# fhausmann/deepgrp

Measured on AMD Instinct MI355X. Metric: Mbp/sec predicted (whole node) at window=200 stride=50, 5-class, higher is better.
Workload: dtype f16

## Files before the change

deepgrp_amd/csrc/api.hip:

```cpp
#include "dgrp_model.h"

#include <stdarg.h>
#include <string.h>

#include <algorithm>
#include <vector>
#include <mutex>

static thread_local char g_err[512] = "";

void dgrp_set_error(const char *fmt, ...)
{
    va_list ap;
    va_start(ap, fmt);
    vsnprintf(g_err, sizeof(g_err), fmt, ap);
    va_end(ap);
}

DGRP_EXPORT int dgrp_abi_version(void) { return DGRP_ABI_VERSION; }
DGRP_EXPORT const char *dgrp_last_error(void) { return g_err; }

DGRP_EXPORT int dgrp_device_info(char *name, size_t name_cap, int *cu_count, int64_t *hbm_bytes)
{
    int dev = 0;
// ... 175 lines not shown
    m->onercp = 0;
    m->UP = (m->u + 31) / 32 * 32; m->NW = m->UP / 32; m->KS = m->UP / 16; m->nfrag = 0;
    m->d_pack = nullptr; m->d_ffb = nullptr; m->d_scale = nullptr; m->d_wtop = nullptr; m->d_raw = nullptr;
    m->d_pack_lo = nullptr; m->precision = 1; m->d_pack16 = nullptr; m->d_xtab = nullptr; m->d_stream = nullptr;
    m->d_packw = nullptr; m->d_xtabw = nullptr; m->NU16 = 0;
    const hipError_t e = upload_raw(m, kernel, rec, bias, nbias, ffk, nffk, ffb, scale);
    if (e != hipSuccess) {
        dgrp_set_error("dgrp_model_create: %s", hipGetErrorString(e));
        dgrp_model_destroy(m);
        return DGRP_EHIP;
    }
    *out = m;
    return DGRP_OK;
}

DGRP_EXPORT int dgrp_model_create(dgrp_model **out, int T, int u, int C, int attention, const float *kernel,
                                  const float *rec, const float *bias, const float *scale, const float *ffk,
                                  const float *ffb)
{
    DGRP_REQUIRE(out, "dgrp_model_create: NULL out");
    *out = nullptr;
    DGRP_REQUIRE(T >= 1 && T <= 65535, "dgrp_model_create: window size %d out of range", T);
    DGRP_REQUIRE(u >= 1 && u <= 2048, "dgrp_model_create: units=%d not supported (1..2048)", u);
    DGRP_REQUIRE(C >= 2 && C <= DGRP_MAXC, "dgrp_model_create: classes=%d not supported (2..%d)", C, DGRP_MAXC);
    DGRP_REQUIRE(kernel && rec && bias && ffk && ffb && (!attention || scale), "dgrp_model_create: NULL tensor");
    char nm[8];
    int rc = dgrp_device_info(nm, sizeof(nm), nullptr, nullptr);
    if (rc != DGRP_OK) return rc;

    dgrp_model *m = new dgrp_model();
    m->T = T; m->u = u; m->C = C; m->attention = attention ? 1 : 0;
    m->cell = 0;
    m->ref_only = 0; m->is_view = 0;
    if (u > 256 || C > 16) return create_ref_only(out, m, kernel, rec, bias, 2 * 3 * (int64_t)u, ffk, (int64_t)(attention ? 2 : 1) * u * C, ffb,
                                        attention ? scale : nullptr);
    m->UP = (u + 31) / 32 * 32;
    m->NW = m->UP / 32;
    m->KS = m->UP / 16;
    m->nfrag = 3 * (m->KS + 1) + 3;
    m->d_pack = nullptr; m->d_ffb = nullptr; m->d_scale = nullptr; m->d_wtop = nullptr; m->d_raw = nullptr;
    m->d_pack_lo = nullptr; m->precision = 0; m->d_pack16 = nullptr; m->d_xtab = nullptr; m->d_stream = nullptr;
    m->d_packw = nullptr; m->d_xtabw = nullptr; m->NU16 = 0;
    const int KS = m->KS, NF = m->nfrag, u3 = 3 * u;
    {
        double worst = 0.0;
        for (int j = 0; j < u; ++j) {
            double bz = 1.0, bg = 0.0;
            double kz = 0.0, kg = 0.0;
            for (int c = 0; c < 5; ++c) {
                kz = std::max(kz, (double)fabsf(kernel[(size_t)c * u3 + j]));
                kg = std::max(kg, (double)fabsf(kernel[(size_t)c * u3 + 2 * u + j]));
            }
            double sz = kz + fabs((double)bias[j] + (double)bias[u3 + j]);
            double sg = kg + fabsf(bias[2 * u + j]) + fabsf(bias[u3 + 2 * u + j]);
            for (int k = 0; k < u; ++k) {
                sz += fabsf(rec[(size_t)k * u3 + j]);
                sg += fabsf(rec[(size_t)k * u3 + 2 * u + j]);
            }
            bz += 1.4426950408889634 * sz;
            bg += 2.8853900817779268 * sg;
            if (!(bz + bg <= worst)) worst = bz + bg;
        }
        const char *safe = getenv("DGRP_GRU_SAFE");
        m->onercp = (m->NW <= 4 && worst <= 120.0 && !(safe && safe[0] == '1')) ? 1 : 0;
    }

    std::vector<uint16_t> pack((size_t)m->NW * NF * 64 * 8, 0);
    frag_writer fw{ pack, NF };
    for (int w = 0; w < m->NW; ++w) {
        for (int l = 0; l < 64; ++l) {
            const int unit = 32 * w + (l & 31);
            const bool uok = unit < u;
            for (int g = 0; g < 3; ++g) {
                const float gs = g < 2 ? -1.4426950408889634f : 2.8853900817779268f;
                pack_recurrent(fw, w, l, g * (KS + 1), KS, rec, u3, g * u + unit, u, uok, gs);
                float v8[8] = { 0, 0, 0, 0, 0, 0, 0, 0 };
                if (uok) {
                    for (int j = 0; j < 5; ++j) v8[j] = g < 2 ? gs * kernel[(size_t)j * u3 + g * u + unit] : 0.0f;
                    v8[5] = gs * (g < 2 ? (float)((double)bias[g * u + unit] + (double)bias[u3 + g * u + unit]) : bias[u3 + 2 * u + unit]);
                    if (m->onercp && g == 0) v8[5] += 1.0f;
                }
                pack_input(fw, w, l, g * (KS + 1) + KS, v8);
            }
            float x8[8] = { 0, 0, 0, 0, 0, 0, 0, 0 };
            if (uok) {
                for (int j = 0; j < 5; ++j) x8[j] = 2.8853900817779268f * kernel[(size_t)j * u3 + 2 * u + unit];
                x8[5] = 2.8853900817779268f * bias[2 * u + unit];
            }
            pack_input(fw, w, l, 3 * (KS + 1), x8);
            pack_dense(fw, w, l, 3 * (KS + 1) + 1, 3 * (KS + 1) + 2, ffk, attention ? u : 0, u, C);
        }
    }
    float ffb16[16] = { 0 };
    for (int c = 0; c < C; ++c) ffb16[c] = ffb[c];

#define CREATE_HIP(call)                                                                   \
    do {                                                                                   \
        hipError_t e_ = (call);                                                            \
        if (e_ != hipSuccess) {                                                            \
            dgrp_set_error("%s failed: %s", #call, hipGetErrorString(e_));                 \
            dgrp_model_destroy(m);                                                         \
            return DGRP_EHIP;                                                              \
        }                                                                                  \
    } while (0)
    CREATE_HIP(hipMalloc((void **)&m->d_pack, pack.size() * 2));
    CREATE_HIP(hipMemcpy(m->d_pack, pack.data(), pack.size() * 2, hipMemcpyHostToDevice));
    CREATE_HIP(hipMalloc((void **)&m->d_ffb, sizeof(ffb16)));
    CREATE_HIP(hipMemcpy(m->d_ffb, ffb16, sizeof(ffb16), hipMemcpyHostToDevice));
    if (attention) {
        std::vector<float> sc(m->UP, 0.0f), wtop((size_t)m->UP * 16, 0.0f);
        for (int k = 0; k < u; ++k) {
            sc[k] = scale[k];
            for (int c = 0; c < C; ++c) wtop[(size_t)k * 16 + c] = ffk[(size_t)k * C + c];
        }
        CREATE_HIP(hipMalloc((void **)&m->d_scale, sc.size() * 4));
        CREATE_HIP(hipMemcpy(m->d_scale, sc.data(), sc.size() * 4, hipMemcpyHostToDevice));
        CREATE_HIP(hipMalloc((void **)&m->d_wtop, wtop.size() * 4));
        CREATE_HIP(hipMemcpy(m->d_wtop, wtop.data(), wtop.size() * 4, hipMemcpyHostToDevice));
    }
    CREATE_HIP(upload_raw(m, kernel, rec, bias, 2 * (int64_t)u3, ffk, (int64_t)(attention ? 2 : 1) * u * C, ffb,
                          attention ? scale : nullptr));
    if (m->NW <= 4) {
        std::vector<uint16_t> lo((size_t)m->NW * 3 * KS * 64 * 8, 0);
        static const int order[3] = { 1, 2, 0 };
        for (int w = 0; w < m->NW; ++w)
            for (int ks = 0; ks < KS; ++ks)
                for (int gi = 0; gi < 3; ++gi) {
                    const int g = order[gi];
                    const float gs = g < 2 ? -1.4426950408889634f : 2.8853900817779268f;
                    for (int l = 0; l < 64; ++l) {
                        const int unit = 32 * w + (l & 31);
                        for (int j = 0; j < 8; ++j) {
                            const int k = 16 * ks + 8 * (l >> 5) + j;
                            uint16_t v = 0;
                            if (unit < u && k < u) {
                                const float x = gs * rec[(size_t)k * u3 + g * u + unit];
                                v = f2h(x - h2f(f2h(x)));
                            }
                            lo[((((size_t)w * KS + ks) * 3 + gi) * 64 + l) * 8 + j] = v;
                        }
                    }
            }
        CREATE_HIP(hipMalloc((void **)&m->d_pack_lo, lo.size() * 2));
        CREATE_HIP(hipMemcpy(m->d_pack_lo, lo.data(), lo.size() * 2, hipMemcpyHostToDevice));
        if (m->NW == 4) {
            static const int order16[3] = { 1, 2, 0 };
            std::vector<uint16_t> p16((size_t)4 * 48 * 64 * 8, 0);
            for (int w = 0; w < 4; ++w)
                for (int gi = 0; gi < 3; ++gi)
                    for (int ks = 0; ks < 4; ++ks)
                        for (int uh = 0; uh < 2; ++uh)
                            for (int l = 0; l < 64; ++l)
                                for (int j = 0; j < 8; ++j) {
                                    const int g = order16[gi], unit = 32 * w + 16 * uh + (l & 15), k = 32 * ks + 8 * (l >> 4) + j;
                                    uint16_t hi = 0, lo16 = 0;
                                    if (unit < u && k < u) {
                                        const float gs = g < 2 ? -1.4426950408889634f : 2.8853900817779268f;
                                        const float x = gs * rec[(size_t)k * u3 + g * u + unit];
                                        hi = f2h(x);
                                        lo16 = f2h(x - h2f(hi));
                                    }
                                    const size_t f = (size_t)gi * 8 + ks * 2 + uh;
                                    p16[(((size_t)w * 48 + f) * 64 + l) * 8 + j] = hi;
                                    p16[(((size_t)w * 48 + 24 + f) * 64 + l) * 8 + j] = lo16;
                                }
            std::vector<float> xt((size_t)5 * 4 * 128, 0.0f);
            const double cs = -1.4426950408889634, ch = 2.8853900817779268;
            for (int b = 0; b < 5; ++b)
                for (int unit = 0; unit < u; ++unit) {
                    float *row = &xt[(size_t)b * 512];
                    row[0 * 128 + unit] = (float)(cs * ((double)kernel[(size_t)b * u3 + u + unit] + (double)bias[u + unit] + (double)bias[u3 + u + unit]));
                    row[1 * 128 + unit] = (float)(ch * (double)bias[u3 + 2 * u + unit]);
                    row[2 * 128 + unit] = (float)(cs * ((double)kernel[(size_t)b * u3 + unit] + (double)bias[unit] + (double)bias[u3 + unit]) + (m->onercp ? 1.0 : 0.0));
                    row[3 * 128 + unit] = (float)(ch * ((double)kernel[(size_t)b * u3 + 2 * u + unit] + (double)bias[2 * u + unit]));
                }
            CREATE_HIP(hipMalloc((void **)&m->d_pack16, p16.size() * 2));
            CREATE_HIP(hipMemcpy(m->d_pack16, p16.data(), p16.size() * 2, hipMemcpyHostToDevice));
            CREATE_HIP(hipMalloc((void **)&m->d_xtab, xt.size() * 4));
            CREATE_HIP(hipMemcpy(m->d_xtab, xt.data(), xt.size() * 4, hipMemcpyHostToDevice));
        }
        if (u <= 64) {
            const int NU = (u + 15) / 16, KSw = (NU + 1) / 2, UP16 = 16 * NU, NFw = 6 * KSw * NU;
            auto wave_col = [](int c) { const int j = c / 32, q = (c % 32) / 8, sub = c % 8; return 16 * (2 * j + (sub >= 4 ? 1 : 0)) + 4 * q + (sub & 3); };
            static const int orderw[3] = { 1, 2, 0 };
            std::vector<uint16_t> pw((size_t)(NFw + 2 * KSw) * 64 * 8, 0);
            for (int gi = 0; gi < 3; ++gi)
                for (int ks = 0; ks < KSw; ++ks)
                    for (int ug = 0; ug < NU; ++ug)
                        for (int l = 0; l < 64; ++l)
                            for (int j = 0; j < 8; ++j) {
                                const int g = orderw[gi], unit = 16 * ug + (l & 15), k = wave_col(32 * ks + 8 * (l >> 4) + j);
                                if (unit >= u || k >= u) continue;
                                const float gs = g < 2 ? -1.4426950408889634f : 2.8853900817779268f;
                                const float x = gs * rec[(size_t)k * u3 + g * u + unit];
                                const uint16_t hi = f2h(x);
                                pw[((size_t)((gi * KSw + ks) * NU + ug) * 64 + l) * 8 + j] = hi;
                                pw[((size_t)(((3 + gi) * KSw + ks) * NU + ug) * 64 + l) * 8 + j] = f2h(x - h2f(hi));
                            }
            const int drow0 = attention ? u : 0;
            for (int ks = 0; ks < KSw; ++ks)
                for (int l = 0; l < 64; ++l)
                    for (int j = 0; j < 8; ++j) {
                        const int k = wave_col(32 * ks + 8 * (l >> 4) + j), c = l & 15;
                        if (k >= u || c >= C) continue;
                        const float v = 0.5f * ffk[(size_t)(drow0 + k) * C + c];
                        const uint16_t hi = f2h(v);
                        pw[((size_t)(NFw + 2 * ks) * 64 + l) * 8 + j] = hi;
                        pw[((size_t)(NFw + 2 * ks + 1) * 64 + l) * 8 + j] = f2h(v - h2f(hi));
                    }
            std::vector<float> xt((size_t)5 * 4 * UP16, 0.0f);
            const double cs = -1.4426950408889634, ch = 2.8853900817779268;
            for (int b = 0; b < 5; ++b)
                for (int unit = 0; unit < u; ++unit) {
                    float *row = &xt[(size_t)b * 4 * UP16];
                    row[0 * UP16 + unit] = (float)(cs * ((double)kernel[(size_t)b * u3 + u + unit] + (double)bias[u + unit] + (double)bias[u3 + u + unit]));
                    row[1 * UP16 + unit] = (float)(ch * (double)bias[u3 + 2 * u + unit]);
                    row[2 * UP16 + unit] = (float)(cs * ((double)kernel[(size_t)b * u3 + unit] + (double)bias[unit] + (double)bias[u3 + unit]) + (m->onercp ? 1.0 : 0.0));
                    row[3 * UP16 + unit] = (float)(ch * ((double)kernel[(size_t)b * u3 + 2 * u + unit] + (double)bias[2 * u + unit]));
                }
            CREATE_HIP(hipMalloc((void **)&m->d_packw, pw.size() * 2));
            CREATE_HIP(hipMemcpy(m->d_packw, pw.data(), pw.size() * 2, hipMemcpyHostToDevice));
            CREATE_HIP(hipMalloc((void **)&m->d_xtabw, xt.size() * 4));
            CREATE_HIP(hipMemcpy(m->d_xtabw, xt.data(), xt.size() * 4, hipMemcpyHostToDevice));
            m->NU16 = NU;
        }
        const char *pe = getenv("DGRP_GRU_PRECISION");
        m->precision = !(pe && pe[0] == '0') ? 1 : 0;
    }
    if (m->NW > 4) {
        static const float gs3[3] = { -1.4426950408889634f, -1.4426950408889634f, 2.8853900817779268f };
        CREATE_HIP(upload_stream(m, rec, 3, gs3));
        {
            const int UPm = m->UP;
            std::vector<float> xt((size_t)5 * 4 * UPm, 0.0f);
            const double cs = -1.4426950408889634, ch = 2.8853900817779268;
            for (int b = 0; b < 5; ++b)
                for (int unit = 0; unit < u; ++unit) {
                    float *row = &xt[(size_t)b * 4 * UPm];
                    row[0 * UPm + unit] = (float)(cs * ((double)kernel[(size_t)b * u3 + u + unit] + (double)bias[u + unit] + (double)bias[u3 + u + unit]));
                    row[1 * UPm + unit] = (float)(ch * (double)bias[u3 + 2 * u + unit]);
                    row[2 * UPm + unit] = (float)(cs * ((double)kernel[(size_t)b * u3 + unit] + (double)bias[unit] + (double)bias[u3 + unit]));
                    row[3 * UPm + unit] = (float)(ch * ((double)kernel[(size_t)b * u3 + 2 * u + unit] + (double)bias[2 * u + unit]));
                }
            CREATE_HIP(hipMalloc((void **)&m->d_xtab, xt.size() * 4));
            CREATE_HIP(hipMemcpy(m->d_xtab, xt.data(), xt.size() * 4, hipMemcpyHostToDevice));
        }
        const char *pe = getenv("DGRP_GRU_PRECISION");
        m->precision = !(pe && pe[0] == '0') ? 1 : 0;
    }
#undef CREATE_HIP
    *out = m;
    return DGRP_OK;
}

DGRP_EXPORT int dgrp_model_create_lstm(dgrp_model **out, int T, int u, int C, const float *kernel, const float *rec,
                                       const float *bias, const float *ffk, const float *ffb)
{
    DGRP_REQUIRE(out, "dgrp_model_create_lstm: NULL out");
    *out = nullptr;
    DGRP_REQUIRE(T >= 1 && T <= 65535, "dgrp_model_create_lstm: window size %d out of range", T);
    DGRP_REQUIRE(u >= 1 && u <= 2048, "dgrp_model_create_lstm: units=%d not supported (1..2048)", u);
    DGRP_REQUIRE(C >= 2 && C <= DGRP_MAXC, "dgrp_model_create_lstm: classes=%d not supported (2..%d)", C, DGRP_MAXC);
    DGRP_REQUIRE(kernel && rec && bias && ffk && ffb, "dgrp_model_create_lstm: NULL tensor");
    char nm[8];
    int rc = dgrp_device_info(nm, sizeof(nm), nullptr, nullptr);
    if (rc != DGRP_OK) return rc;
    dgrp_model *m = new dgrp_model();
    m->T = T; m->u = u; m->C = C; m->attention = 0; m->cell = 1;
    m->ref_only = 0; m->is_view = 0;
    if (u > 256 || C > 16) return create_ref_only(out, m, kernel, rec, bias, 4 * (int64_t)u, ffk, (int64_t)u * C, ffb, nullptr);
    m->UP = (u + 31) / 32 * 32;
    m->NW = m->UP / 32;
    m->KS = m->UP / 16;
    m->nfrag = 4 * (m->KS + 1) + 2;
    m->d_pack = nullptr; m->d_ffb = nullptr; m->d_scale = nullptr; m->d_wtop = nullptr; m->d_raw = nullptr;
    m->d_pack_lo = nullptr; m->precision = 0; m->d_pack16 = nullptr; m->d_xtab = nullptr; m->d_stream = nullptr;
    m->d_packw = nullptr; m->d_xtabw = nullptr; m->NU16 = 0;
    const int KS = m->KS, NF = m->nfrag, u4 = 4 * u;
    std::vector<uint16_t> pack((size_t)m->NW * NF * 64 * 8, 0);
    frag_writer fw{ pack, NF };
    for (int w = 0; w < m->NW; ++w)
        for (int l = 0; l < 64; ++l) {
            const int unit = 32 * w + (l & 31);
            const bool uok = unit < u;
            for (int g = 0; g < 4; ++g) {
                const float gs = g == 2 ? 2.8853900817779268f : -1.4426950408889634f;
                pack_recurrent(fw, w, l, g * (KS + 1), KS, rec, u4, g * u + unit, u, uok, gs);
                float v8[8] = { 0, 0, 0, 0, 0, 0, 0, 0 };
                if (uok) {
                    for (int j = 0; j < 5; ++j) v8[j] = gs * kernel[(size_t)j * u4 + g * u + unit];
                    v8[5] = gs * bias[g * u + unit];
                }
                pack_input(fw, w, l, g * (KS + 1) + KS, v8);
            }
            pack_dense(fw, w, l, 4 * (KS + 1), 4 * (KS + 1) + 1, ffk, 0, u, C);
        }
    float ffb16[16] = { 0 };
    for (int c = 0; c < C; ++c) ffb16[c] = ffb[c];
    hipError_t e = hipMalloc((void **)&m->d_pack, pack.size() * 2);
    if (e == hipSuccess) e = hipMemcpy(m->d_pack, pack.data(), pack.size() * 2, hipMemcpyHostToDevice);
    if (e == hipSuccess) e = hipMalloc((void **)&m->d_ffb, sizeof(ffb16));
    if (e == hipSuccess) e = hipMemcpy(m->d_ffb, ffb16, sizeof(ffb16), hipMemcpyHostToDevice);
    if (e == hipSuccess) e = upload_raw(m, kernel, rec, bias, u4, ffk, (int64_t)u * C, ffb, nullptr);
    if (e == hipSuccess) {
        static const float gs4[4] = { -1.4426950408889634f, -1.4426950408889634f, 2.8853900817779268f, -1.4426950408889634f };
        e = upload_stream(m, rec, 4, gs4);
        const char *pe = getenv("DGRP_GRU_PRECISION");
// ... 528 lines not shown
```

deepgrp_amd/csrc/gru_split2.hip:

```cpp
#include "gru_shared.h"
#include <mutex>
#include <type_traits>

typedef unsigned u32x4 __attribute__((ext_vector_type(4)));

namespace {

constexpr int NW = 4, UP = 128, KS = 4, HPAD = 16, HS = UP + HPAD;
constexpr int XT_PITCH = 4 * 128 * 4 + 32;

struct split2_weights {
    u32x4 hi[3][KS][2], lo[3][KS][2];
    u32x4 Bd_hi, Bd_lo;
};

#define LOAD2(a, pa, b, pb)                                                                                             \
    asm volatile("global_load_dwordx4 %0, %2, off\n\tglobal_load_dwordx4 %1, %3, off\n\ts_waitcnt vmcnt(0)"            \
                 : "=&a"(a), "=&a"(b) : "v"(pa), "v"(pb) : "memory")

#define MFMA_R(acc, Wf, b) asm volatile("v_mfma_f32_16x16x32_f16 %0, %1, %2, %0" : "+v"(acc) : "a"(Wf), "v"(b))
#define MFMA_D(acc, a, Wf) asm volatile("v_mfma_f32_16x16x32_f16 %0, %1, %2, %0" : "+v"(acc) : "v"(a), "a"(Wf))
#define MFMA_DZ(acc, a, Wf) asm volatile("v_mfma_f32_16x16x32_f16 %0, %1, %2, 0" : "=&v"(acc) : "v"(a), "a"(Wf))

struct tile_state {
    gru_params p;
    wg_ctx ctx;
    unsigned hcur, hnxt, lcur, lnxt;
    unsigned myseq;
    float h[16];
    f32x4 ar[4], ag[4], az[4], ax[4];
    f32x4 dpl;
    unsigned tabf, tabr;
    half8 f0h[2], f0l[2];
    int p_off;
    int64_t p_row0;
    bool pr_on;
};

template <int MODE, bool ONERCP>
__global__ void __launch_bounds__(256) __attribute__((amdgpu_waves_per_eu(1, 1))) gru_split2_kernel(const gru_params pin, int half_bytes)
{
    extern __shared__ __attribute__((aligned(16))) unsigned char smem[];
    const int tid = threadIdx.x;
    const int lane = tid & 63;
    const int wave = __builtin_amdgcn_readfirstlane(tid >> 6);
    const int T = pin.T, C = pin.C;

    split2_weights W;
    {
        const uint4 *p16 = pin.pack16 + (size_t)wave * 48 * 64 + lane;
#pragma unroll
        for (int g = 0; g < 3; ++g)
#pragma unroll
            for (int ks = 0; ks < KS; ++ks) {
                LOAD2(W.hi[g][ks][0], p16 + (size_t)(g * 8 + ks * 2) * 64, W.hi[g][ks][1], p16 + (size_t)(g * 8 + ks * 2 + 1) * 64);
                LOAD2(W.lo[g][ks][0], p16 + (size_t)(24 + g * 8 + ks * 2) * 64, W.lo[g][ks][1], p16 + (size_t)(24 + g * 8 + ks * 2 + 1) * 64);
            }
        const uint4 *mypack = pin.pack + (size_t)wave * pin.nfrag * 64 + lane;
        LOAD2(W.Bd_hi, mypack + (size_t)(3 * (2 * KS + 1) + 1) * 64, W.Bd_lo, mypack + (size_t)(3 * (2 * KS + 1) + 2) * 64);
    }
    for (int i = tid; i < 5 * 512; i += 256)
        *reinterpret_cast<float *>(smem + pin.xtab_off + (i / 512) * XT_PITCH + (i % 512) * 4) = pin.xtab[i];

    const int wi = lane & 15, q4 = lane >> 4;
    const int cls = lane & 15;
    const float fbias = cls < C ? pin.ffb[cls] : 0.0f;
    const int pwi = 4 * (lane >> 4) + wave;
    const unsigned frag_lane = (unsigned)(wi * HS + 8 * q4) * 2;
    const unsigned dense_lane = (unsigned)(wi * HS + 32 * wave + 8 * q4) * 2;
    const unsigned pub_lane = (unsigned)(wi * HS + 32 * wave + 4 * q4) * 2;
    const unsigned tab_lane = (unsigned)pin.xtab_off + (unsigned)(32 * wave + 4 * q4) * 4;

    tile_state S0, S1;
    auto setup = [&](tile_state &Z, int x) {
        unsigned char *base = smem + (size_t)x * half_bytes;
        _Float16 *lbuf = reinterpret_cast<_Float16 *>(base + pin.lo_tile_off);
        for (int i = tid; i < 32 * HS; i += 256) lbuf[i] = (_Float16)0.0f;
        Z.p = pin;
        const int64_t bid = wg_record_at<MODE>(pin, Z.p, 2 * (int64_t)blockIdx.x + x);
        Z.ctx = wg_setup<NW, MODE, HPAD>(Z.p, base, bid);
        Z.hcur = (unsigned)x * half_bytes;
        Z.hnxt = Z.hcur + 32 * HS * 2;
        Z.lcur = (unsigned)x * half_bytes + pin.lo_tile_off;
        Z.lnxt = Z.lcur + 32 * HS * 2;
        Z.myseq = (unsigned)(Z.ctx.seqs - smem) + wi * pin.Tp;
#pragma unroll
        for (int i = 0; i < 16; ++i) Z.h[i] = ONERCP ? -1.0f : 0.0f;
        Z.p_off = Z.ctx.rowoff[pwi];
        Z.p_row0 = Z.ctx.row0s[pwi];
        Z.pr_on = cls < C && pwi < Z.ctx.nvalid;
    };
    setup(S0, 0);
    setup(S1, 1);

    auto lds16 = [&](unsigned off) -> half8 { return *reinterpret_cast<const half8 *>(smem + off); };
    auto ldsf4 = [&](unsigned off) -> f32x4 { return *reinterpret_cast<const f32x4 *>(smem + off); };
    auto tab_rows = [&](tile_state &Z, uint32_t bf, uint32_t br) {
        bf = bf < 4 ? bf : 4;
        br = br < 4 ? 3 - br : 4;
        Z.tabf = tab_lane + bf * XT_PITCH;
        Z.tabr = tab_lane + br * XT_PITCH;
    };
    auto acc_init = [&](tile_state &Z, int g, int sub) {
        const f32x4 v = ldsf4(((sub & 1) ? Z.tabr : Z.tabf) + g * 512 + (sub >> 1) * 64);
        if (g == 0) Z.ar[sub] = v; else if (g == 1) Z.ag[sub] = v; else Z.az[sub] = v;
    };

    struct frag_ring { half8 h[2][2], l[2][2]; };
    struct dense_ops { half8 a0, a1, l0, l1; };
    struct fin_state { float d[NW], lg, m, e, s; };
    auto phase = [&](auto do_x, auto do_y, auto do_f, tile_state &X, tile_state &Y, int tx, int ty) __attribute__((always_inline)) {
        constexpr bool DO_X = decltype(do_x)::value, DO_Y = decltype(do_y)::value, DO_F = decltype(do_f)::value;
        frag_ring F;
        dense_ops D;
        fin_state fs;
        split_gate_tmp gt[16];
        float pbh[4][4];
        uint2 pbhv[4], pblv[4];
        uint32_t xp_bf = 4, xp_br = 4;
        const int td = ty - 1;
        const int tf = tx - 2;
        if constexpr (DO_X) { F.h[0][0] = X.f0h[0]; F.h[0][1] = X.f0h[1]; F.l[0][0] = X.f0l[0]; F.l[0][1] = X.f0l[1]; }
#define GAP __builtin_amdgcn_sched_barrier(0);
#define M_K(ks, n)                                                                                               \
    if constexpr (DO_X) {                                                                                        \
        constexpr int ps_ = (n) / 12, g_ = ((n) % 12) / 4, uh_ = ((n) % 4) / 2, rh_ = (n) % 2, sub_ = 2 * uh_ + rh_; \
        const half8 &b_ = ps_ == 1 ? F.l[(ks) & 1][rh_] : F.h[(ks) & 1][rh_];                                    \
        const u32x4 &w_ = ps_ == 2 ? W.lo[g_][ks][uh_] : W.hi[g_][ks][uh_];                                      \
        if constexpr (g_ == 0) MFMA_R(X.ar[sub_], w_, b_);                                                       \
        else if constexpr (g_ == 1) MFMA_R(X.ag[sub_], w_, b_);                                                  \
        else MFMA_R(X.az[sub_], w_, b_);                                                                         \
    }
#define M_D(i)                                                                                                   \
    if constexpr (DO_X) {                                                                                        \
        if constexpr ((i) == 0) MFMA_DZ(X.dpl, D.a0, W.Bd_hi);                                                   \
        else if constexpr ((i) == 1) MFMA_D(X.dpl, D.a1, W.Bd_hi);                                               \
        else if constexpr ((i) == 2) MFMA_D(X.dpl, D.a0, W.Bd_lo);                                               \
        else if constexpr ((i) == 3) MFMA_D(X.dpl, D.a1, W.Bd_lo);                                               \
        else if constexpr ((i) == 4) MFMA_D(X.dpl, D.l0, W.Bd_hi);                                               \
        else MFMA_D(X.dpl, D.l1, W.Bd_hi);                                                                       \
    }
#define PF(ks)                                                                                                   \
    if constexpr (DO_X) {                                                                                        \
        F.h[(ks) & 1][0] = lds16(X.hcur + frag_lane + 64 * (ks)); F.h[(ks) & 1][1] = lds16(X.hcur + frag_lane + 16 * HS * 2 + 64 * (ks)); \
        F.l[(ks) & 1][0] = lds16(X.lcur + frag_lane + 64 * (ks)); F.l[(ks) & 1][1] = lds16(X.lcur + frag_lane + 16 * HS * 2 + 64 * (ks)); \
    }
#define RDD                                                                                                      \
    if constexpr (DO_X) {                                                                                        \
        D.a0 = lds16(X.hcur + dense_lane); D.a1 = lds16(X.hcur + dense_lane + 16 * HS * 2);                      \
        D.l0 = lds16(X.lcur + dense_lane); D.l1 = lds16(X.lcur + dense_lane + 16 * HS * 2);                      \
        if (MODE == 2 && tx > 0 && (lane & 15) < X.ctx.nvalid)                                                   \
            split_avg_store(X.p, X.ctx.wg_w, tx - 1, UP, wave, D.a0, D.a1, D.l0, D.l1);                          \
    }
#define AXL(sub) \
    if constexpr (DO_Y) Y.ax[sub] = ldsf4((((sub) & 1) ? Y.tabr : Y.tabf) + 3 * 512 + ((sub) >> 1) * 64);
#define DS(i)                                                                                                    \
    if constexpr (DO_Y) Y.ctx.dpart[((size_t)(td & 1) * 4 * NW + wave) * 64 + lane + (i) * NW * 64] = Y.dpl[i];
#define G(e, op) \
    if constexpr (DO_Y) split_gate_op<ONERCP, op>(gt[e], Y.ar[(e) / 4][(e) % 4], Y.ag[(e) / 4][(e) % 4], Y.az[(e) / 4][(e) % 4], Y.ax[(e) / 4][(e) % 4], Y.h[e]);
#define PB(g, op)                                                                                                \
    if constexpr (DO_Y) {                                                                                        \
        if constexpr ((op) == 0) {                                                                               \
            pbh[g][0] = split_state_h<ONERCP>(Y.h[4 * (g)]); pbh[g][1] = split_state_h<ONERCP>(Y.h[4 * (g) + 1]); \
            pbh[g][2] = split_state_h<ONERCP>(Y.h[4 * (g) + 2]); pbh[g][3] = split_state_h<ONERCP>(Y.h[4 * (g) + 3]); \
        } else if constexpr ((op) == 1) {                                                                        \
            pbhv[g] = split_pack4(pbh[g]);                                                                       \
        } else if constexpr ((op) == 2) {                                                                        \
            split_residual4(pbh[g], pbhv[g]);                                                                    \
        } else if constexpr ((op) == 3) {                                                                        \
            pblv[g] = split_pack4(pbh[g]);                                                                       \
        } else {                                                                                                 \
            *reinterpret_cast<uint2 *>(smem + Y.hnxt + pub_lane + ((g) & 1) * 16 * HS * 2 + ((g) >> 1) * 32) = pbhv[g]; \
            *reinterpret_cast<uint2 *>(smem + Y.lnxt + pub_lane + ((g) & 1) * 16 * HS * 2 + ((g) >> 1) * 32) = pblv[g]; \
        }                                                                                                        \
    }
#define BAR                                                                                                      \
    if constexpr (DO_Y) {                                                                                        \
        asm volatile("s_waitcnt lgkmcnt(0)\n\ts_barrier" ::: "memory");                                          \
        unsigned sw_ = Y.hcur; Y.hcur = Y.hnxt; Y.hnxt = sw_;                                                    \
        sw_ = Y.lcur; Y.lcur = Y.lnxt; Y.lnxt = sw_;                                                             \
    }
#define RD0                                                                                                      \
    if constexpr (DO_Y) {                                                                                        \
        Y.f0h[0] = lds16(Y.hcur + frag_lane); Y.f0h[1] = lds16(Y.hcur + frag_lane + 16 * HS * 2);                \
        Y.f0l[0] = lds16(Y.lcur + frag_lane); Y.f0l[1] = lds16(Y.lcur + frag_lane + 16 * HS * 2);                \
    }
#define XP(op)                                                                                                   \
    if constexpr (DO_Y) {                                                                                        \
        if constexpr ((op) == 0) { xp_bf = smem[Y.myseq + ty + 1]; xp_br = smem[Y.myseq + T - 2 - ty]; }                       \
        else tab_rows(Y, xp_bf, xp_br);                                                                          \
    }
#define CI(g, sub) \
    if constexpr (DO_Y) acc_init(Y, g, sub);
#define FN(op)                                                                                                   \
    if constexpr (DO_F) {                                                                                        \
        if constexpr ((op) == 0) {                                                                               \
            const float *dp_ = X.ctx.dpart + ((size_t)(tf & 1) * 4 + wave) * NW * 64 + lane;                     \
            fs.d[0] = dp_[0]; fs.d[1] = dp_[64]; fs.d[2] = dp_[128]; fs.d[3] = dp_[192];                         \
        } else if constexpr ((op) == 1) {                                                                        \
            const float sum_ = ((fs.d[0] + fs.d[1]) + fs.d[2]) + fs.d[3];                                        \
            fs.lg = cls < C ? sum_ + fbias : -INFINITY;                                                          \
        } else if constexpr ((op) == 2) { if (MODE != 2) fs.m = row_max_ror<8>(fs.lg); }                         \
        else if constexpr ((op) == 3) { if (MODE != 2) fs.m = row_max_ror<4>(fs.m); }                            \
        else if constexpr ((op) == 4) { if (MODE != 2) fs.m = row_max_ror<2>(fs.m); }                            \
        else if constexpr ((op) == 5) { if (MODE != 2) fs.m = row_max_ror<1>(fs.m); }                            \
        else if constexpr ((op) == 6) { if (MODE != 2) fs.e = __builtin_amdgcn_exp2f(1.4426950408889634f * (fs.lg - fs.m)); } \
        else if constexpr ((op) == 7) { if (MODE != 2) fs.s = fs.e + row_ror<8>(fs.e); }                         \
        else if constexpr ((op) == 8) { if (MODE != 2) fs.s += row_ror<4>(fs.s); }                               \
        else if constexpr ((op) == 9) { if (MODE != 2) fs.s += row_ror<2>(fs.s); }                               \
        else if constexpr ((op) == 10) { if (MODE != 2) fs.s += row_ror<1>(fs.s); }                              \
        else if constexpr ((op) == 11) { if (MODE != 2) fs.e *= __builtin_amdgcn_rcpf(fs.s); }                   \
        else { if (X.pr_on && tf >= 0) emit_value<MODE>(X.p, X.ctx, X.p_off, X.p_row0, tf, cls, MODE == 2 ? fs.lg : fs.e); } \
    }
#include "gru_split2_phase.inc"
#undef GAP
#undef M_K
#undef M_D
#undef PF
#undef RDD
#undef AXL
#undef DS
#undef G
#undef PB
#undef BAR
#undef RD0
#undef XP
#undef CI
#undef FN
    };
    const std::true_type yes;
    const std::false_type no;

    auto first_step = [&](tile_state &Z) {
        tab_rows(Z, smem[Z.myseq], smem[Z.myseq + T - 1]);
#pragma unroll
        for (int g = 0; g < 3; ++g)
#pragma unroll
            for (int sub = 0; sub < 4; ++sub) acc_init(Z, g, sub);
        Z.f0h[0] = lds16(Z.hcur + frag_lane); Z.f0h[1] = lds16(Z.hcur + frag_lane + 16 * HS * 2);
        Z.f0l[0] = lds16(Z.lcur + frag_lane); Z.f0l[1] = lds16(Z.lcur + frag_lane + 16 * HS * 2);
    };
    first_step(S0);
    first_step(S1);
    phase(yes, no, no, S0, S1, 0, 0);
#define EDGE_PAD do { asm volatile("s_nop 15\n\ts_nop 7"); __builtin_amdgcn_sched_barrier(0); } while (0)
    EDGE_PAD;
    for (int t = 0; t + 1 < T; ++t) {
        phase(yes, yes, yes, S1, S0, t, t);
        phase(yes, yes, yes, S0, S1, t + 1, t);
        EDGE_PAD;
    }
    phase(yes, yes, yes, S1, S0, T - 1, T - 1);
    phase(no, yes, yes, S0, S1, T, T - 1);

    auto drain = [&](tile_state &Z, bool prev_open) {
        const half8 a0 = lds16(Z.hcur + dense_lane), a1 = lds16(Z.hcur + dense_lane + 16 * HS * 2);
        const half8 l0 = lds16(Z.lcur + dense_lane), l1 = lds16(Z.lcur + dense_lane + 16 * HS * 2);
        if (MODE == 2 && (lane & 15) < Z.ctx.nvalid) split_avg_store(Z.p, Z.ctx.wg_w, T - 1, UP, wave, a0, a1, l0, l1);
        f32x4 d;
        MFMA_DZ(d, a0, W.Bd_hi); MFMA_D(d, a1, W.Bd_hi); MFMA_D(d, a0, W.Bd_lo); MFMA_D(d, a1, W.Bd_lo); MFMA_D(d, l0, W.Bd_hi); MFMA_D(d, l1, W.Bd_hi);
        asm volatile("s_nop 15\n\ts_nop 7" : "+v"(d));
        float *dw = Z.ctx.dpart + ((size_t)((T - 1) & 1) * 4 * NW + wave) * 64 + lane;
#pragma unroll
        for (int reg = 0; reg < 4; ++reg) dw[reg * NW * 64] = d[reg];
        __syncthreads();
        if (prev_open && T > 1) finish_register<NW, MODE>(Z.p, Z.ctx, T - 2, wave, fbias, Z.p_off, Z.p_row0);
        finish_register<NW, MODE>(Z.p, Z.ctx, T - 1, wave, fbias, Z.p_off, Z.p_row0);
        if (MODE == 0 && pin.ospan > 0) flush_image<NW>(Z.p, Z.ctx);
    };
    drain(S0, false);
    drain(S1, true);
}

template <int MODE, bool ONERCP>
int launch_split2(const gru_params &p, int64_t groups, int half_bytes, hipStream_t stream)
{
    static std::once_flag configured;
    static hipError_t cfg_err = hipSuccess;
    std::call_once(configured, [] { cfg_err = hipFuncSetAttribute((const void *)gru_split2_kernel<MODE, ONERCP>, hipFuncAttributeMaxDynamicSharedMemorySize, 160 * 1024); });
    DGRP_HIP(cfg_err);
    hipLaunchKernelGGL((gru_split2_kernel<MODE, ONERCP>), dim3((unsigned)((groups + 1) / 2)), dim3(256), (size_t)2 * half_bytes + 5 * XT_PITCH, stream, p, half_bytes);
    DGRP_LAUNCH_CHECK();
    return DGRP_OK;
}

}

int dgrp_split2_launch(const gru_params &p, int64_t groups, int half_bytes, bool onercp, hipStream_t stream)
{
    if (onercp)
        return p.mode == 0 ? launch_split2<0, true>(p, groups, half_bytes, stream)
             : p.mode == 1 ? launch_split2<1, true>(p, groups, half_bytes, stream) : launch_split2<2, true>(p, groups, half_bytes, stream);
    return p.mode == 0 ? launch_split2<0, false>(p, groups, half_bytes, stream)
         : p.mode == 1 ? launch_split2<1, false>(p, groups, half_bytes, stream) : launch_split2<2, false>(p, groups, half_bytes, stream);
}
```

deepgrp_amd/csrc/gru_split2_phase.inc:

```
M_K(0, 0) XP(0) RDD GAP
M_K(0, 1) AXL(0) AXL(1) GAP
M_K(0, 2) AXL(2) AXL(3) PF(1) GAP
M_K(0, 3) FN(0) GAP
M_K(0, 4) DS(0) DS(1) DS(2) GAP
M_K(0, 5) DS(3) GAP
M_K(0, 6) G(0, 0) G(0, 1) GAP
M_K(0, 7) G(0, 2) GAP
M_K(0, 8) G(0, 3) G(1, 0) GAP
M_K(0, 9) G(0, 4) GAP
M_K(0, 10) FN(1) GAP
M_K(0, 11) G(1, 1) GAP
M_K(0, 12) XP(1) G(0, 5) G(1, 2) G(0, 6) GAP
M_K(0, 13) G(1, 3) GAP
M_K(0, 14) G(2, 0) G(0, 7) GAP
M_K(0, 15) G(1, 4) GAP
M_K(0, 16) G(2, 1) G(0, 8) GAP
M_K(0, 17) G(1, 5) G(2, 2) G(0, 9) GAP
M_K(0, 18) G(1, 6) GAP
M_K(0, 19) G(2, 3) G(3, 0) GAP
M_K(0, 20) G(0, 10) GAP
M_K(0, 21) G(1, 7) G(2, 4) GAP
M_K(0, 22) G(3, 1) FN(2) GAP
M_K(0, 23) G(0, 11) G(1, 8) GAP
M_D(0) G(2, 5) G(3, 2) GAP
M_K(0, 24) G(1, 9) G(2, 6) GAP
M_K(0, 25) G(3, 3) GAP
M_K(0, 26) G(4, 0) G(1, 10) GAP
M_K(0, 27) G(2, 7) G(3, 4) GAP
M_K(0, 28) CI(0, 0) CI(1, 0) CI(2, 0) GAP
M_K(0, 29) G(4, 1) G(1, 11) GAP
M_K(0, 30) G(2, 8) GAP
M_K(0, 31) G(3, 5) G(4, 2) G(2, 9) GAP
M_K(0, 32) FN(3) GAP
M_K(0, 33) G(3, 6) G(4, 3) GAP
M_K(0, 34) G(5, 0) GAP
M_K(0, 35) G(2, 10) G(3, 7) GAP
M_K(1, 0) G(4, 4) G(5, 1) GAP
M_K(1, 1) G(2, 11) G(3, 8) GAP
M_K(1, 2) PF(2) G(4, 5) G(5, 2) GAP
M_K(1, 3) G(3, 9) G(4, 6) GAP
M_K(1, 4) G(5, 3) GAP
M_K(1, 5) G(6, 0) G(3, 10) GAP
M_K(1, 6) G(4, 7) G(5, 4) GAP
M_K(1, 7) G(6, 1) G(3, 11) GAP
M_K(1, 8) FN(4) GAP
M_K(1, 9) GAP
M_K(1, 10) PB(0, 0) PB(0, 1) GAP
M_K(1, 11) GAP
M_D(1) PB(0, 2) GAP
M_K(1, 12) PB(0, 3) PB(0, 4) GAP
M_K(1, 13) G(4, 8) GAP
M_K(1, 14) G(5, 5) G(6, 2) G(4, 9) GAP
M_K(1, 15) G(5, 6) G(6, 3) GAP
M_K(1, 16) G(7, 0) GAP
M_K(1, 17) G(4, 10) G(5, 7) GAP
M_K(1, 18) G(6, 4) GAP
M_K(1, 19) G(7, 1) G(4, 11) G(5, 8) GAP
M_K(1, 20) G(6, 5) G(7, 2) GAP
M_K(1, 21) FN(5) GAP
M_K(1, 22) G(5, 9) G(6, 6) GAP
M_K(1, 23) G(7, 3) G(8, 0) GAP
M_K(1, 24) G(5, 10) GAP
M_K(1, 25) G(6, 7) G(7, 4) CI(0, 1) GAP
M_K(1, 26) CI(1, 1) CI(2, 1) GAP
M_K(1, 27) G(8, 1) G(5, 11) GAP
M_K(1, 28) G(6, 8) G(7, 5) GAP
M_K(1, 29) G(8, 2) G(6, 9) GAP
M_K(1, 30) G(7, 6) G(8, 3) GAP
M_K(1, 31) G(9, 0) GAP
M_K(1, 32) G(6, 10) G(7, 7) GAP
M_K(1, 33) GAP
M_K(1, 34) FN(6) G(8, 4) GAP
M_K(1, 35) G(9, 1) G(6, 11) GAP
M_D(2) G(7, 8) GAP
M_K(2, 0) G(8, 5) G(9, 2) G(7, 9) GAP
M_K(2, 1) G(8, 6) G(9, 3) GAP
M_K(2, 2) PF(3) G(10, 0) GAP
M_K(2, 3) G(7, 10) G(8, 7) GAP
M_K(2, 4) G(9, 4) G(10, 1) GAP
M_K(2, 5) G(7, 11) GAP
M_K(2, 6) PB(1, 0) GAP
M_K(2, 7) PB(1, 1) GAP
M_K(2, 8) GAP
M_K(2, 9) PB(1, 2) PB(1, 3) GAP
M_K(2, 10) PB(1, 4) GAP
M_K(2, 11) G(8, 8) FN(7) GAP
M_K(2, 12) G(9, 5) GAP
M_K(2, 13) G(10, 2) G(8, 9) G(9, 6) GAP
M_K(2, 14) G(10, 3) GAP
M_K(2, 15) G(11, 0) GAP
M_K(2, 16) G(8, 10) G(9, 7) G(10, 4) GAP
M_K(2, 17) G(11, 1) G(8, 11) GAP
M_K(2, 18) G(9, 8) GAP
M_K(2, 19) G(10, 5) G(11, 2) G(9, 9) GAP
M_K(2, 20) G(10, 6) GAP
M_K(2, 21) G(11, 3) G(12, 0) GAP
M_K(2, 22) G(9, 10) G(10, 7) GAP
M_K(2, 23) G(11, 4) GAP
M_D(3) FN(8) CI(0, 2) CI(1, 2) GAP
M_K(2, 24) CI(2, 2) GAP
M_K(2, 25) G(12, 1) G(9, 11) G(10, 8) GAP
M_K(2, 26) G(11, 5) G(12, 2) GAP
M_K(2, 27) G(10, 9) G(11, 6) GAP
M_K(2, 28) G(12, 3) GAP
M_K(2, 29) G(13, 0) GAP
M_K(2, 30) G(10, 10) G(11, 7) G(12, 4) GAP
M_K(2, 31) G(13, 1) G(10, 11) GAP
M_K(2, 32) G(11, 8) GAP
M_K(2, 33) G(12, 5) G(13, 2) G(11, 9) GAP
M_K(2, 34) FN(9) G(12, 6) GAP
M_K(2, 35) G(13, 3) GAP
M_K(3, 0) G(14, 0) GAP
M_K(3, 1) G(11, 10) G(12, 7) GAP
M_K(3, 2) G(13, 4) G(14, 1) GAP
M_K(3, 3) G(11, 11) GAP
M_K(3, 4) PB(2, 0) GAP
M_K(3, 5) PB(2, 1) GAP
M_K(3, 6) GAP
M_K(3, 7) PB(2, 2) PB(2, 3) GAP
M_K(3, 8) PB(2, 4) G(12, 8) GAP
M_K(3, 9) G(13, 5) GAP
M_K(3, 10) G(14, 2) G(12, 9) G(13, 6) GAP
M_K(3, 11) G(14, 3) GAP
M_D(4) G(15, 0) GAP
M_K(3, 12) G(12, 10) FN(10) GAP
M_K(3, 13) G(13, 7) G(14, 4) GAP
M_K(3, 14) G(15, 1) G(12, 11) GAP
M_K(3, 15) G(13, 8) G(14, 5) GAP
M_K(3, 16) G(15, 2) G(13, 9) GAP
M_K(3, 17) G(14, 6) G(15, 3) GAP
M_K(3, 18) G(13, 10) GAP
M_K(3, 19) G(14, 7) G(15, 4) CI(0, 3) GAP
M_K(3, 20) CI(1, 3) CI(2, 3) G(13, 11) GAP
M_K(3, 21) G(14, 8) GAP
M_K(3, 22) G(15, 5) G(14, 9) G(15, 6) GAP
M_K(3, 23) G(14, 10) GAP
M_D(5) FN(11) GAP
M_K(3, 24) G(15, 7) G(14, 11) G(15, 8) GAP
M_K(3, 25) G(15, 9) GAP
M_K(3, 26) G(15, 10) G(15, 11) GAP
M_K(3, 27) PB(3, 0) GAP
M_K(3, 28) PB(3, 1) GAP
M_K(3, 29) GAP
M_K(3, 30) PB(3, 2) GAP
M_K(3, 31) PB(3, 3) PB(3, 4) BAR GAP
M_K(3, 32) GAP
M_K(3, 33) RD0 GAP
M_K(3, 34) FN(12) GAP
M_K(3, 35) GAP
```

Measured before the change: 538.8.

## Interleave wave unit ownership and reschedule GRU split2 phase to pull barrier earlier

Each wave's hidden units change from a contiguous block of 32 to two interleaved blocks of 16 at offsets 64 apart. The weight packing, table lane offsets, accumulator init strides and publish addresses are all updated to match. The hand-scheduled phase table is reordered so gate work finishes earlier, the final FN steps are batched near the end, and the barrier plus next-fragment read happen a few MFMA slots sooner, shortening the recurrent critical path. New BARA/RD0E macros are defined but not used, and the reordering risks timing or bank-conflict changes in LDS traffic.

```diff
diff --git a/deepgrp_amd/csrc/api.hip b/deepgrp_amd/csrc/api.hip
--- a/deepgrp_amd/csrc/api.hip
+++ b/deepgrp_amd/csrc/api.hip
@@ -351,7 +351,7 @@
                         for (int uh = 0; uh < 2; ++uh)
                             for (int l = 0; l < 64; ++l)
                                 for (int j = 0; j < 8; ++j) {
-                                    const int g = order16[gi], unit = 32 * w + 16 * uh + (l & 15), k = 32 * ks + 8 * (l >> 4) + j;
+                                    const int g = order16[gi], unit = 16 * w + 64 * uh + (l & 15), k = 32 * ks + 8 * (l >> 4) + j;
                                     uint16_t hi = 0, lo16 = 0;
                                     if (unit < u && k < u) {
                                         const float gs = g < 2 ? -1.4426950408889634f : 2.8853900817779268f;
diff --git a/deepgrp_amd/csrc/gru_split2.hip b/deepgrp_amd/csrc/gru_split2.hip
--- a/deepgrp_amd/csrc/gru_split2.hip
+++ b/deepgrp_amd/csrc/gru_split2.hip
@@ -68,8 +68,8 @@
     const int pwi = 4 * (lane >> 4) + wave;
     const unsigned frag_lane = (unsigned)(wi * HS + 8 * q4) * 2;
     const unsigned dense_lane = (unsigned)(wi * HS + 32 * wave + 8 * q4) * 2;
-    const unsigned pub_lane = (unsigned)(wi * HS + 32 * wave + 4 * q4) * 2;
-    const unsigned tab_lane = (unsigned)pin.xtab_off + (unsigned)(32 * wave + 4 * q4) * 4;
+    const unsigned pub_lane = (unsigned)(wi * HS + 16 * wave + 4 * q4) * 2;
+    const unsigned tab_lane = (unsigned)pin.xtab_off + (unsigned)(16 * wave + 4 * q4) * 4;
 
     tile_state S0, S1;
     auto setup = [&](tile_state &Z, int x) {
@@ -102,7 +102,7 @@
         Z.tabr = tab_lane + br * XT_PITCH;
     };
     auto acc_init = [&](tile_state &Z, int g, int sub) {
-        const f32x4 v = ldsf4(((sub & 1) ? Z.tabr : Z.tabf) + g * 512 + (sub >> 1) * 64);
+        const f32x4 v = ldsf4(((sub & 1) ? Z.tabr : Z.tabf) + g * 512 + (sub >> 1) * 256);
         if (g == 0) Z.ar[sub] = v; else if (g == 1) Z.ag[sub] = v; else Z.az[sub] = v;
     };
 
@@ -153,7 +153,7 @@
             split_avg_store(X.p, X.ctx.wg_w, tx - 1, UP, wave, D.a0, D.a1, D.l0, D.l1);                          \
     }
 #define AXL(sub) \
-    if constexpr (DO_Y) Y.ax[sub] = ldsf4((((sub) & 1) ? Y.tabr : Y.tabf) + 3 * 512 + ((sub) >> 1) * 64);
+    if constexpr (DO_Y) Y.ax[sub] = ldsf4((((sub) & 1) ? Y.tabr : Y.tabf) + 3 * 512 + ((sub) >> 1) * 256);
 #define DS(i)                                                                                                    \
     if constexpr (DO_Y) Y.ctx.dpart[((size_t)(td & 1) * 4 * NW + wave) * 64 + lane + (i) * NW * 64] = Y.dpl[i];
 #define G(e, op) \
@@ -170,8 +170,8 @@
         } else if constexpr ((op) == 3) {                                                                        \
             pblv[g] = split_pack4(pbh[g]);                                                                       \
         } else {                                                                                                 \
-            *reinterpret_cast<uint2 *>(smem + Y.hnxt + pub_lane + ((g) & 1) * 16 * HS * 2 + ((g) >> 1) * 32) = pbhv[g]; \
-            *reinterpret_cast<uint2 *>(smem + Y.lnxt + pub_lane + ((g) & 1) * 16 * HS * 2 + ((g) >> 1) * 32) = pblv[g]; \
+            *reinterpret_cast<uint2 *>(smem + Y.hnxt + pub_lane + ((g) & 1) * 16 * HS * 2 + ((g) >> 1) * 128) = pbhv[g]; \
+            *reinterpret_cast<uint2 *>(smem + Y.lnxt + pub_lane + ((g) & 1) * 16 * HS * 2 + ((g) >> 1) * 128) = pblv[g]; \
         }                                                                                                        \
     }
 #define BAR                                                                                                      \
@@ -184,6 +184,16 @@
     if constexpr (DO_Y) {                                                                                        \
         Y.f0h[0] = lds16(Y.hcur + frag_lane); Y.f0h[1] = lds16(Y.hcur + frag_lane + 16 * HS * 2);                \
         Y.f0l[0] = lds16(Y.lcur + frag_lane); Y.f0l[1] = lds16(Y.lcur + frag_lane + 16 * HS * 2);                \
+    }
+#define BARA                                                                                                     \
+    if constexpr (DO_Y) {                                                                                        \
+        asm volatile("s_waitcnt lgkmcnt(0)\n\ts_barrier" ::: "memory");                                          \
+        __builtin_amdgcn_sched_barrier(0);                                                                       \
+    }
+#define RD0E                                                                                                     \
+    if constexpr (DO_Y) {                                                                                        \
+        Y.f0h[0] = lds16(Y.hnxt + frag_lane); Y.f0h[1] = lds16(Y.hnxt + frag_lane + 16 * HS * 2);                \
+        Y.f0l[0] = lds16(Y.lnxt + frag_lane); Y.f0l[1] = lds16(Y.lnxt + frag_lane + 16 * HS * 2);                \
     }
 #define XP(op)                                                                                                   \
     if constexpr (DO_Y) {                                                                                        \
@@ -223,6 +233,8 @@
 #undef G
 #undef PB
 #undef BAR
+#undef BARA
+#undef RD0E
 #undef RD0
 #undef XP
 #undef CI
diff --git a/deepgrp_amd/csrc/gru_split2_phase.inc b/deepgrp_amd/csrc/gru_split2_phase.inc
--- a/deepgrp_amd/csrc/gru_split2_phase.inc
+++ b/deepgrp_amd/csrc/gru_split2_phase.inc
@@ -7,144 +7,144 @@
 M_K(0, 6) G(0, 0) G(0, 1) GAP
 M_K(0, 7) G(0, 2) GAP
 M_K(0, 8) G(0, 3) G(1, 0) GAP
-M_K(0, 9) G(0, 4) GAP
-M_K(0, 10) FN(1) GAP
-M_K(0, 11) G(1, 1) GAP
-M_K(0, 12) XP(1) G(0, 5) G(1, 2) G(0, 6) GAP
-M_K(0, 13) G(1, 3) GAP
-M_K(0, 14) G(2, 0) G(0, 7) GAP
-M_K(0, 15) G(1, 4) GAP
-M_K(0, 16) G(2, 1) G(0, 8) GAP
-M_K(0, 17) G(1, 5) G(2, 2) G(0, 9) GAP
-M_K(0, 18) G(1, 6) GAP
-M_K(0, 19) G(2, 3) G(3, 0) GAP
-M_K(0, 20) G(0, 10) GAP
-M_K(0, 21) G(1, 7) G(2, 4) GAP
-M_K(0, 22) G(3, 1) FN(2) GAP
-M_K(0, 23) G(0, 11) G(1, 8) GAP
-M_D(0) G(2, 5) G(3, 2) GAP
-M_K(0, 24) G(1, 9) G(2, 6) GAP
-M_K(0, 25) G(3, 3) GAP
-M_K(0, 26) G(4, 0) G(1, 10) GAP
-M_K(0, 27) G(2, 7) G(3, 4) GAP
-M_K(0, 28) CI(0, 0) CI(1, 0) CI(2, 0) GAP
-M_K(0, 29) G(4, 1) G(1, 11) GAP
-M_K(0, 30) G(2, 8) GAP
-M_K(0, 31) G(3, 5) G(4, 2) G(2, 9) GAP
-M_K(0, 32) FN(3) GAP
-M_K(0, 33) G(3, 6) G(4, 3) GAP
-M_K(0, 34) G(5, 0) GAP
-M_K(0, 35) G(2, 10) G(3, 7) GAP
-M_K(1, 0) G(4, 4) G(5, 1) GAP
-M_K(1, 1) G(2, 11) G(3, 8) GAP
-M_K(1, 2) PF(2) G(4, 5) G(5, 2) GAP
-M_K(1, 3) G(3, 9) G(4, 6) GAP
-M_K(1, 4) G(5, 3) GAP
-M_K(1, 5) G(6, 0) G(3, 10) GAP
-M_K(1, 6) G(4, 7) G(5, 4) GAP
-M_K(1, 7) G(6, 1) G(3, 11) GAP
-M_K(1, 8) FN(4) GAP
+M_K(0, 9) G(0, 4) G(1, 1) GAP
+M_K(0, 10) G(0, 5) GAP
+M_K(0, 11) G(1, 2) G(0, 6) GAP
+M_K(0, 12) XP(1) G(1, 3) GAP
+M_K(0, 13) G(2, 0) G(0, 7) G(1, 4) GAP
+M_K(0, 14) G(2, 1) G(0, 8) GAP
+M_K(0, 15) G(1, 5) GAP
+M_K(0, 16) G(2, 2) G(0, 9) G(1, 6) GAP
+M_K(0, 17) G(2, 3) GAP
+M_K(0, 18) G(3, 0) GAP
+M_K(0, 19) G(0, 10) G(1, 7) G(2, 4) GAP
+M_K(0, 20) G(3, 1) GAP
+M_K(0, 21) G(0, 11) G(1, 8) GAP
+M_K(0, 22) G(2, 5) G(3, 2) G(1, 9) GAP
+M_K(0, 23) G(2, 6) GAP
+M_D(0) G(3, 3) G(4, 0) GAP
+M_K(0, 24) GAP
+M_K(0, 25) FN(1) GAP
+M_K(0, 26) G(1, 10) G(2, 7) G(3, 4) GAP
+M_K(0, 27) CI(0, 0) CI(1, 0) GAP
+M_K(0, 28) CI(2, 0) G(4, 1) GAP
+M_K(0, 29) G(1, 11) G(2, 8) GAP
+M_K(0, 30) G(3, 5) G(4, 2) GAP
+M_K(0, 31) G(2, 9) G(3, 6) GAP
+M_K(0, 32) G(4, 3) GAP
+M_K(0, 33) G(5, 0) G(2, 10) GAP
+M_K(0, 34) G(3, 7) G(4, 4) GAP
+M_K(0, 35) G(5, 1) G(2, 11) GAP
+M_K(1, 0) G(3, 8) G(4, 5) GAP
+M_K(1, 1) G(5, 2) G(3, 9) GAP
+M_K(1, 2) PF(2) G(4, 6) G(5, 3) GAP
+M_K(1, 3) G(6, 0) GAP
+M_K(1, 4) G(3, 10) G(4, 7) GAP
+M_K(1, 5) G(5, 4) G(6, 1) GAP
+M_K(1, 6) G(3, 11) GAP
+M_K(1, 7) PB(0, 0) GAP
+M_K(1, 8) PB(0, 1) GAP
 M_K(1, 9) GAP
-M_K(1, 10) PB(0, 0) PB(0, 1) GAP
-M_K(1, 11) GAP
-M_D(1) PB(0, 2) GAP
-M_K(1, 12) PB(0, 3) PB(0, 4) GAP
-M_K(1, 13) G(4, 8) GAP
-M_K(1, 14) G(5, 5) G(6, 2) G(4, 9) GAP
-M_K(1, 15) G(5, 6) G(6, 3) GAP
-M_K(1, 16) G(7, 0) GAP
-M_K(1, 17) G(4, 10) G(5, 7) GAP
-M_K(1, 18) G(6, 4) GAP
-M_K(1, 19) G(7, 1) G(4, 11) G(5, 8) GAP
-M_K(1, 20) G(6, 5) G(7, 2) GAP
-M_K(1, 21) FN(5) GAP
-M_K(1, 22) G(5, 9) G(6, 6) GAP
-M_K(1, 23) G(7, 3) G(8, 0) GAP
-M_K(1, 24) G(5, 10) GAP
-M_K(1, 25) G(6, 7) G(7, 4) CI(0, 1) GAP
-M_K(1, 26) CI(1, 1) CI(2, 1) GAP
-M_K(1, 27) G(8, 1) G(5, 11) GAP
-M_K(1, 28) G(6, 8) G(7, 5) GAP
-M_K(1, 29) G(8, 2) G(6, 9) GAP
-M_K(1, 30) G(7, 6) G(8, 3) GAP
-M_K(1, 31) G(9, 0) GAP
-M_K(1, 32) G(6, 10) G(7, 7) GAP
-M_K(1, 33) GAP
-M_K(1, 34) FN(6) G(8, 4) GAP
-M_K(1, 35) G(9, 1) G(6, 11) GAP
-M_D(2) G(7, 8) GAP
-M_K(2, 0) G(8, 5) G(9, 2) G(7, 9) GAP
-M_K(2, 1) G(8, 6) G(9, 3) GAP
-M_K(2, 2) PF(3) G(10, 0) GAP
-M_K(2, 3) G(7, 10) G(8, 7) GAP
-M_K(2, 4) G(9, 4) G(10, 1) GAP
-M_K(2, 5) G(7, 11) GAP
-M_K(2, 6) PB(1, 0) GAP
-M_K(2, 7) PB(1, 1) GAP
-M_K(2, 8) GAP
-M_K(2, 9) PB(1, 2) PB(1, 3) GAP
-M_K(2, 10) PB(1, 4) GAP
-M_K(2, 11) G(8, 8) FN(7) GAP
-M_K(2, 12) G(9, 5) GAP
-M_K(2, 13) G(10, 2) G(8, 9) G(9, 6) GAP
-M_K(2, 14) G(10, 3) GAP
-M_K(2, 15) G(11, 0) GAP
-M_K(2, 16) G(8, 10) G(9, 7) G(10, 4) GAP
-M_K(2, 17) G(11, 1) G(8, 11) GAP
-M_K(2, 18) G(9, 8) GAP
-M_K(2, 19) G(10, 5) G(11, 2) G(9, 9) GAP
-M_K(2, 20) G(10, 6) GAP
-M_K(2, 21) G(11, 3) G(12, 0) GAP
-M_K(2, 22) G(9, 10) G(10, 7) GAP
-M_K(2, 23) G(11, 4) GAP
-M_D(3) FN(8) CI(0, 2) CI(1, 2) GAP
-M_K(2, 24) CI(2, 2) GAP
-M_K(2, 25) G(12, 1) G(9, 11) G(10, 8) GAP
-M_K(2, 26) G(11, 5) G(12, 2) GAP
-M_K(2, 27) G(10, 9) G(11, 6) GAP
-M_K(2, 28) G(12, 3) GAP
-M_K(2, 29) G(13, 0) GAP
-M_K(2, 30) G(10, 10) G(11, 7) G(12, 4) GAP
-M_K(2, 31) G(13, 1) G(10, 11) GAP
-M_K(2, 32) G(11, 8) GAP
-M_K(2, 33) G(12, 5) G(13, 2) G(11, 9) GAP
-M_K(2, 34) FN(9) G(12, 6) GAP
-M_K(2, 35) G(13, 3) GAP
-M_K(3, 0) G(14, 0) GAP
-M_K(3, 1) G(11, 10) G(12, 7) GAP
-M_K(3, 2) G(13, 4) G(14, 1) GAP
-M_K(3, 3) G(11, 11) GAP
-M_K(3, 4) PB(2, 0) GAP
-M_K(3, 5) PB(2, 1) GAP
-M_K(3, 6) GAP
-M_K(3, 7) PB(2, 2) PB(2, 3) GAP
-M_K(3, 8) PB(2, 4) G(12, 8) GAP
-M_K(3, 9) G(13, 5) GAP
-M_K(3, 10) G(14, 2) G(12, 9) G(13, 6) GAP
-M_K(3, 11) G(14, 3) GAP
-M_D(4) G(15, 0) GAP
-M_K(3, 12) G(12, 10) FN(10) GAP
-M_K(3, 13) G(13, 7) G(14, 4) GAP
-M_K(3, 14) G(15, 1) G(12, 11) GAP
-M_K(3, 15) G(13, 8) G(14, 5) GAP
-M_K(3, 16) G(15, 2) G(13, 9) GAP
-M_K(3, 17) G(14, 6) G(15, 3) GAP
-M_K(3, 18) G(13, 10) GAP
-M_K(3, 19) G(14, 7) G(15, 4) CI(0, 3) GAP
-M_K(3, 20) CI(1, 3) CI(2, 3) G(13, 11) GAP
-M_K(3, 21) G(14, 8) GAP
-M_K(3, 22) G(15, 5) G(14, 9) G(15, 6) GAP
-M_K(3, 23) G(14, 10) GAP
-M_D(5) FN(11) GAP
-M_K(3, 24) G(15, 7) G(14, 11) G(15, 8) GAP
-M_K(3, 25) G(15, 9) GAP
-M_K(3, 26) G(15, 10) G(15, 11) GAP
-M_K(3, 27) PB(3, 0) GAP
-M_K(3, 28) PB(3, 1) GAP
-M_K(3, 29) GAP
-M_K(3, 30) PB(3, 2) GAP
-M_K(3, 31) PB(3, 3) PB(3, 4) BAR GAP
+M_K(1, 10) PB(0, 2) PB(0, 3) GAP
+M_K(1, 11) PB(0, 4) GAP
+M_D(1) G(4, 8) G(5, 5) GAP
+M_K(1, 12) G(6, 2) G(4, 9) G(5, 6) GAP
+M_K(1, 13) G(6, 3) GAP
+M_K(1, 14) G(7, 0) GAP
+M_K(1, 15) G(4, 10) G(5, 7) GAP
+M_K(1, 16) G(6, 4) G(7, 1) GAP
+M_K(1, 17) G(4, 11) G(5, 8) GAP
+M_K(1, 18) G(6, 5) G(7, 2) GAP
+M_K(1, 19) G(5, 9) G(6, 6) GAP
+M_K(1, 20) G(7, 3) GAP
+M_K(1, 21) G(8, 0) G(5, 10) GAP
+M_K(1, 22) G(6, 7) G(7, 4) CI(0, 1) GAP
+M_K(1, 23) CI(1, 1) CI(2, 1) GAP
+M_K(1, 24) G(8, 1) G(5, 11) GAP
+M_K(1, 25) G(6, 8) GAP
+M_K(1, 26) G(7, 5) G(8, 2) G(6, 9) GAP
+M_K(1, 27) G(7, 6) G(8, 3) GAP
+M_K(1, 28) G(9, 0) GAP
+M_K(1, 29) G(6, 10) G(7, 7) GAP
+M_K(1, 30) G(8, 4) GAP
+M_K(1, 31) G(9, 1) FN(2) GAP
+M_K(1, 32) G(6, 11) G(7, 8) GAP
+M_K(1, 33) G(8, 5) G(9, 2) GAP
+M_K(1, 34) G(7, 9) G(8, 6) GAP
+M_K(1, 35) G(9, 3) G(10, 0) GAP
+M_D(2) G(7, 10) GAP
+M_K(2, 0) G(8, 7) G(9, 4) GAP
+M_K(2, 1) G(10, 1) G(7, 11) GAP
+M_K(2, 2) PF(3) GAP
+M_K(2, 3) PB(1, 0) PB(1, 1) GAP
+M_K(2, 4) GAP
+M_K(2, 5) PB(1, 2) GAP
+M_K(2, 6) PB(1, 3) GAP
+M_K(2, 7) PB(1, 4) G(8, 8) GAP
+M_K(2, 8) G(9, 5) G(10, 2) G(8, 9) GAP
+M_K(2, 9) G(9, 6) GAP
+M_K(2, 10) G(10, 3) G(11, 0) GAP
+M_K(2, 11) G(8, 10) GAP
+M_K(2, 12) G(9, 7) G(10, 4) GAP
+M_K(2, 13) G(11, 1) G(8, 11) G(9, 8) GAP
+M_K(2, 14) G(10, 5) GAP
+M_K(2, 15) G(11, 2) G(9, 9) G(10, 6) GAP
+M_K(2, 16) G(11, 3) GAP
+M_K(2, 17) G(12, 0) GAP
+M_K(2, 18) G(9, 10) G(10, 7) G(11, 4) GAP
+M_K(2, 19) CI(0, 2) CI(1, 2) GAP
+M_K(2, 20) CI(2, 2) G(12, 1) GAP
+M_K(2, 21) G(9, 11) G(10, 8) GAP
+M_K(2, 22) G(11, 5) G(12, 2) GAP
+M_K(2, 23) G(10, 9) G(11, 6) GAP
+M_D(3) G(12, 3) GAP
+M_K(2, 24) G(13, 0) G(10, 10) GAP
+M_K(2, 25) G(11, 7) G(12, 4) GAP
+M_K(2, 26) G(13, 1) G(10, 11) GAP
+M_K(2, 27) G(11, 8) G(12, 5) GAP
+M_K(2, 28) G(13, 2) G(11, 9) GAP
+M_K(2, 29) G(12, 6) G(13, 3) GAP
+M_K(2, 30) G(14, 0) GAP
+M_K(2, 31) G(11, 10) G(12, 7) GAP
+M_K(2, 32) G(13, 4) G(14, 1) GAP
+M_K(2, 33) G(11, 11) GAP
+M_K(2, 34) PB(2, 0) GAP
+M_K(2, 35) PB(2, 1) GAP
+M_K(3, 0) GAP
+M_K(3, 1) PB(2, 2) PB(2, 3) GAP
+M_K(3, 2) PB(2, 4) GAP
+M_K(3, 3) G(12, 8) G(13, 5) GAP
+M_K(3, 4) FN(3) G(14, 2) GAP
+M_K(3, 5) G(12, 9) G(13, 6) GAP
+M_K(3, 6) G(14, 3) GAP
+M_K(3, 7) G(15, 0) GAP
+M_K(3, 8) G(12, 10) G(13, 7) G(14, 4) GAP
+M_K(3, 9) G(15, 1) G(12, 11) GAP
+M_K(3, 10) G(13, 8) GAP
+M_K(3, 11) G(14, 5) G(15, 2) G(13, 9) GAP
+M_D(4) G(14, 6) GAP
+M_K(3, 12) G(15, 3) G(13, 10) GAP
+M_K(3, 13) G(14, 7) G(15, 4) CI(0, 3) GAP
+M_K(3, 14) CI(1, 3) CI(2, 3) GAP
+M_K(3, 15) G(13, 11) G(14, 8) GAP
+M_K(3, 16) G(15, 5) G(14, 9) G(15, 6) GAP
+M_K(3, 17) G(14, 10) GAP
+M_K(3, 18) G(15, 7) G(14, 11) G(15, 8) GAP
+M_K(3, 19) G(15, 9) GAP
+M_K(3, 20) G(15, 10) G(15, 11) GAP
+M_K(3, 21) PB(3, 0) GAP
+M_K(3, 22) PB(3, 1) GAP
+M_K(3, 23) GAP
+M_D(5) PB(3, 2) GAP
+M_K(3, 24) PB(3, 3) PB(3, 4) GAP
+M_K(3, 25) FN(4) FN(5) GAP
+M_K(3, 26) FN(6) FN(7) GAP
+M_K(3, 27) FN(8) FN(9) GAP
+M_K(3, 28) FN(10) FN(11) GAP
+M_K(3, 29) BAR RD0 GAP
+M_K(3, 30) GAP
+M_K(3, 31) FN(12) GAP
 M_K(3, 32) GAP
-M_K(3, 33) RD0 GAP
-M_K(3, 34) FN(12) GAP
+M_K(3, 33) GAP
+M_K(3, 34) GAP
 M_K(3, 35) GAP
```

After: 541.6 (median of 6 runs). Within noise of the previous version (+0.5%).
